# od-liu/CS3602-LLM-Inference-Acceleration

Measured on NVIDIA B200. Metric: kv_compress_step_throughput, higher is better.
Workload: dtype bf16

## Files before the change

### cs3602-llm-inference-acceleration_b200/csrc/kvc_device.cuh

```cuda
#pragma once
#include <cuda_bf16.h>
#include <cuda_fp16.h>
#include <cuda_runtime.h>
#include <stdint.h>

#include <type_traits>

#include "kvc.h"

namespace kvc {

constexpr int kHistBits = 11;
constexpr int kHistBins = 1 << kHistBits;
constexpr int kMiscInts = 128;
constexpr int kMaxPoolHalo = 32;

constexpr int kMiscBin = 0;
constexpr int kMiscBelow = 1;
constexpr int kMiscMaxRaw = 2;
constexpr int kMiscWarpA = 32;
constexpr int kMiscWarpB = 64;
constexpr int kMiscHalo = 96;

struct CarryDev {
    char* acc;
    int64_t asb, ash;
    int32_t group, prev;
};
static_assert(sizeof(CarryDev) == 32, "CarryDev is part of the kernel parameters");

struct LayerDev {
    const char* k_in;
    const char* v_in;
    char* k_out;
    char* v_out;
    int32_t* idx_out;
    const int32_t* idx_in;
    int64_t ksb, ksh, kss;
    int64_t vsb, vsh, vss;
    int32_t S, sink, lo, hi, ksel, tail, score, pool;
    const char* n_in;
    int64_t nsb, nsh;
    CarryDev carry;
};
static_assert(sizeof(LayerDev) == 184, "LayerDev is passed by value in kernel params");

struct BatchDev {
    int32_t B, H;
    int32_t idx_cap;
    int32_t cpr;
    int32_t pad0, pad1;
    int32_t nsw;
    int32_t off_hist, off_idx, off_keys, off_stage;
    int32_t upc;
    char* ws;
    int64_t ws_unit;
    int64_t ws_keys;
    LayerDev layers[KVC_MAX_LAYERS_PER_LAUNCH];
};
static_assert(sizeof(BatchDev) < 32 * 1024, "kernel parameters are limited to 32 KB");

template <int DT>
struct Traits;
template <>
struct Traits<KVC_DTYPE_F32> {
    using Key = uint32_t;
    static constexpr int kElemBytes = 4;
    static constexpr int kKeyBits = 32;
    __device__ static __forceinline__ uint32_t to_raw(float x) { return __float_as_uint(x); }
    __device__ static __forceinline__ float from_raw(uint32_t r) { return __uint_as_float(r); }
    __device__ static __forceinline__ float sumsq(int4 v, float acc) {
        float a = __int_as_float(v.x), b = __int_as_float(v.y), c = __int_as_float(v.z), d = __int_as_float(v.w);
        acc = fmaf(a, a, acc);
        acc = fmaf(b, b, acc);
        acc = fmaf(c, c, acc);
        acc = fmaf(d, d, acc);
        return acc;
    }
};
template <>
struct Traits<KVC_DTYPE_BF16> {
    using Key = uint16_t;
    static constexpr int kElemBytes = 2;
    static constexpr int kKeyBits = 16;
    __device__ static __forceinline__ uint32_t to_raw(float x) {
        return (uint32_t)__bfloat16_as_ushort(__float2bfloat16_rn(x));
    }
    __device__ static __forceinline__ float from_raw(uint32_t r) { return __uint_as_float(r << 16); }
    __device__ static __forceinline__ float sumsq(int4 v, float acc) {
        const uint32_t w[4] = {(uint32_t)v.x, (uint32_t)v.y, (uint32_t)v.z, (uint32_t)v.w};
#pragma unroll
        for (int i = 0; i < 4; ++i) {
            float lo = __uint_as_float(w[i] << 16);
            float hi = __uint_as_float(w[i] & 0xffff0000u);
            acc = fmaf(lo, lo, acc);
            acc = fmaf(hi, hi, acc);
        }
        return acc;
    }
};
template <>
struct Traits<KVC_DTYPE_F16> {
    using Key = uint16_t;
    static constexpr int kElemBytes = 2;
    static constexpr int kKeyBits = 16;
    __device__ static __forceinline__ uint32_t to_raw(float x) {
        return (uint32_t)__half_as_ushort(__float2half_rn(x));
    }
    __device__ static __forceinline__ float from_raw(uint32_t r) {
        return __half2float(__ushort_as_half((unsigned short)r));
    }
    __device__ static __forceinline__ float sumsq(int4 v, float acc) {
        const uint32_t w[4] = {(uint32_t)v.x, (uint32_t)v.y, (uint32_t)v.z, (uint32_t)v.w};
#pragma unroll
        for (int i = 0; i < 4; ++i) {
            float lo = __half2float(__ushort_as_half((unsigned short)(w[i] & 0xffffu)));
            float hi = __half2float(__ushort_as_half((unsigned short)(w[i] >> 16)));
            acc = fmaf(lo, lo, acc);
            acc = fmaf(hi, hi, acc);
        }
        return acc;
    }
};

template <int DT>
__device__ __forceinline__ float round_dt(float x) {
    return Traits<DT>::from_raw(Traits<DT>::to_raw(x));
}

template <typename Key>
__device__ __forceinline__ Key ordered_key(uint32_t raw, bool descending) {
    constexpr int kBits = sizeof(Key) * 8;
    const uint32_t sign = (raw >> (kBits - 1)) & 1u;
    uint32_t k = sign ? ~raw : (raw | (1u << (kBits - 1)));
    if (descending) k = ~k;
    return (Key)k;
}

__device__ __forceinline__ int4 ldg128_stream(const void* p) {
    int4 r;
    asm volatile("ld.global.nc.L1::no_allocate.v4.s32 {%0,%1,%2,%3}, [%4];"
                 : "=r"(r.x), "=r"(r.y), "=r"(r.z), "=r"(r.w)
                 : "l"(p));
    return r;
}
__device__ __forceinline__ void stg128_stream(void* p, int4 v) {
    asm volatile("st.global.L1::no_allocate.v4.s32 [%0], {%1,%2,%3,%4};" ::"l"(p), "r"(v.x), "r"(v.y), "r"(v.z),
                 "r"(v.w)
                 : "memory");
}

__device__ __forceinline__ float group_sum_pow2(float v, int n) {
    for (int o = n >> 1; o > 0; o >>= 1) v += __shfl_xor_sync(0xffffffffu, v, o);
    return v;
}

template <int NT>
__device__ __forceinline__ void find_bin(const uint32_t* hist, int nbins, uint32_t k, int32_t* misc) {
    const int tid = threadIdx.x, lane = tid & 31, warp = tid >> 5;
    const int per = (nbins + NT - 1) / NT;
    const int b0 = tid * per;
    uint32_t loc = 0;
    if ((per & 3) == 0) {
        for (int i = 0; i < per; i += 4) {
            if (b0 + i < nbins) {
                uint4 h = *reinterpret_cast<const uint4*>(hist + b0 + i);
                loc += h.x + h.y + h.z + h.w;
            }
        }
    } else {
        for (int i = 0; i < per; ++i)
            if (b0 + i < nbins) loc += hist[b0 + i];
    }
    uint32_t inc = loc;
#pragma unroll
    for (int o = 1; o < 32; o <<= 1) {
        uint32_t t = __shfl_up_sync(0xffffffffu, inc, o);
        if (lane >= o) inc += t;
    }
    if (lane == 31) misc[kMiscWarpA + warp] = (int32_t)inc;
    __syncthreads();
    uint32_t wbase = 0;
    for (int w = 0; w < warp; ++w) wbase += (uint32_t)misc[kMiscWarpA + w];
    const uint32_t excl = wbase + inc - loc;
    if (excl < k && k <= excl + loc) {
        uint32_t c = excl;
        for (int i = 0; i < per; ++i) {
            const uint32_t h = hist[b0 + i];
            if (c + h >= k) {
                misc[kMiscBin] = b0 + i;
                misc[kMiscBelow] = (int32_t)c;
                break;
            }
            c += h;
        }
    }
    __syncthreads();
}

template <typename Key, int NT>
__device__ __forceinline__ void block_radix_select(const Key* __restrict__ keys, int R, int k, uint32_t* hist,
                                                   int32_t* misc, int32_t* out_idx, int base) {
    constexpr int kBits = sizeof(Key) * 8;
    constexpr int kVec = 16 / sizeof(Key);
// ... 322 lines not shown
```

### cs3602-llm-inference-acceleration_b200/csrc/kvc_fused_tma.cuh

```cuda
#pragma once
#include "kvc_device.cuh"
#include "kvc_tma.cuh"

namespace kvc {

__host__ __device__ constexpr int swz_bits(int cpr) { return (cpr % 8 == 0) ? 3 : (cpr % 4 == 0) ? 2 : (cpr % 2 == 0) ? 1 : 0; }

template <int DT, int CPR>
__device__ __forceinline__ float row_sumsq_smem(uint32_t row_addr, int lane, int cpr) {
    using Tr = Traits<DT>;
    if constexpr (CPR == 0) {
        float tot = 0.f;
        for (int c = 0; c < cpr; ++c) {
            const float a = Tr::sumsq(lds128(row_addr + c * 16), 0.f);
            tot = (c == 0) ? a : tot + a;
        }
        return tot;
    } else {
        constexpr int SB = swz_bits(CPR);
        constexpr int G = 1 << SB;
        const int x = (lane >> (3 - SB)) & (G - 1);
        uint32_t base[G];
#pragma unroll
        for (int m = 0; m < G; ++m) base[m] = row_addr + (uint32_t)(((m ^ x) - m) * 16);
        float acc[CPR];
#pragma unroll
        for (int c = 0; c < CPR; ++c) acc[c] = Tr::sumsq(lds128(base[c & (G - 1)] + c * 16), 0.f);
        float tot = 0.f;
#pragma unroll
        for (int g = 0; g < CPR / G; ++g) {
#pragma unroll
            for (int s = 1; s < G; s <<= 1) {
#pragma unroll
                for (int m = 0; m < G; m += 2 * s) acc[g * G + m] += acc[g * G + m + s];
            }
            tot = (g == 0) ? acc[0] : tot + acc[g * G];
        }
        return tot;
    }
}

__device__ __forceinline__ void warp_load_rows(uint32_t slot, uint32_t bar, const char* src, int rows, bool dense,
                                               int lane, int rb) {
    const bool in = lane < rows;
    const unsigned long long a = (unsigned long long)src;
    const unsigned long long prev = __shfl_up_sync(0xffffffffu, a, 1);
    const bool head = in && (lane == 0 || !dense || a != prev + (unsigned)rb);
    const uint32_t heads = __ballot_sync(0xffffffffu, head);
    if (lane == 0) mbar_arrive_expect_tx(bar, (uint32_t)(rows * rb));
    __syncwarp();
    if (head) {
        const uint32_t later = heads & ~((2u << lane) - 1u);
        const int next = later ? (__ffs(later) - 1) : rows;
        bulk_g2s(slot + (uint32_t)(lane * rb), src, (uint32_t)((next - lane) * rb), bar);
    }
}

struct KeepMap {
    const int32_t* sidx;
    int sink, ksel, tail0;
    __device__ __forceinline__ int operator()(int j) const {
        return j < sink ? j : (j < sink + ksel ? sidx[j - sink] : j + tail0);
    }
};

template <typename Key, int NT>
__device__ __forceinline__ void carry_unit(const CarryDev& c, const KeepMap& src_row, int C, int b, int h) {
    char* base = c.acc + (int64_t)b * c.asb + (int64_t)h * c.group * c.ash;
    const int n = c.group * C;
    for (int e0 = 0; e0 < n; e0 += NT) {
        const int e = e0 + (int)threadIdx.x;
        Key* row = nullptr;
        int i = 0;
        Key val = 0;
        bool write = false;
        if (e < n) {
            const int g = e / C;
            i = e - g * C;
            const int s = src_row(i);
            row = reinterpret_cast<Key*>(base + (int64_t)g * c.ash);
            write = s != i || s >= c.prev;
            if (write && s < c.prev) val = row[s];
        }
        __syncthreads();
        if (write) row[i] = val;
    }
}

__device__ __forceinline__ void gather_unit(const KeepMap& src_row, int C, const char* kbase, const char* vbase,
                                            int64_t kss, int64_t vss, char* ko, char* vo, int rb, uint32_t slot,
                                            uint32_t bar, uint32_t& parity, int stage, int nstage, int lane) {
    const bool kdense = kss == rb, vdense = vss == rb;
    const int nbc = (C + 31) >> 5;
    for (int t = stage; t < 2 * nbc; t += nstage) {
        const bool isv = t >= nbc;
        const int j0 = (isv ? t - nbc : t) << 5;
        const int rows = min(32, C - j0);
        const int row = lane < rows ? src_row(j0 + lane) : 0;
        const char* src = isv ? vbase + (int64_t)row * vss : kbase + (int64_t)row * kss;
        warp_load_rows(slot, bar, src, rows, isv ? vdense : kdense, lane, rb);
        mbar_wait(bar, parity);
        parity ^= 1;
        if (lane == 0) {
            bulk_s2g((isv ? vo : ko) + (int64_t)j0 * rb, slot, (uint32_t)(rows * rb));
            bulk_commit();
            bulk_wait_read<0>();
        }
        __syncwarp();
    }
}

template <int DT, int NT>
__device__ __forceinline__ void keys_from_values(const typename Traits<DT>::Key* src, int R, int score,
                                                 typename Traits<DT>::Key* keys, uint32_t* hist, int32_t* misc) {
    using Tr = Traits<DT>;
    using Key = typename Tr::Key;
    constexpr int kShift0 = Tr::kKeyBits - kHistBits;
    const bool snap = (score == KVC_SCORE_SNAPKV_POOL);
    const bool desc = (score == KVC_SCORE_L2_HIGH);
    uint32_t local_max = 0;
    load_keys_vectorised<DT, NT>(src, R, keys, [&](int i, uint32_t raw) {
        if (snap) {
            keys[i] = (Key)raw;
            local_max = max(local_max, raw);
        } else {
            const Key key = ordered_key<Key>(raw, desc);
            keys[i] = key;
            atomicAdd(&hist[(uint32_t)key >> kShift0], 1u);
        }
    });
    if (snap) {
#pragma unroll
        for (int o = 16; o > 0; o >>= 1) local_max = max(local_max, __shfl_xor_sync(0xffffffffu, local_max, o));
        if ((threadIdx.x & 31) == 0) atomicMax(reinterpret_cast<uint32_t*>(&misc[kMiscMaxRaw]), local_max);
    }
}

template <int DT, int NT, typename Layer>
__device__ __forceinline__ void select_from_memory(const Layer& L, const typename Traits<DT>::Key* norm_row, int b, int bh,
                                                   typename Traits<DT>::Key* keys, uint32_t* hist, int32_t* misc,
                                                   int32_t* sidx) {
    using Key = typename Traits<DT>::Key;
    const int tid = threadIdx.x;
    const int R = L.hi - L.lo;
    if (L.score == KVC_SCORE_GIVEN_INDEX) {
        const int32_t* src = L.idx_in + (int64_t)bh * L.ksel;
        for (int i = tid; i < L.ksel; i += NT) sidx[i] = min(max(src[i], 0), L.S - 1);
        return;
    }
    for (int i = tid; i < kHistBins; i += NT) hist[i] = 0;
    if (tid == 0) misc[kMiscMaxRaw] = 0;
    __syncthreads();
    if (L.score == KVC_SCORE_GIVEN_SCORE || L.score == KVC_SCORE_GIVEN_SCORE_SHARED) {
        const Key* src = reinterpret_cast<const Key*>(L.idx_in) + (int64_t)(L.score == KVC_SCORE_GIVEN_SCORE ? bh : b) * R;
        load_keys_vectorised<DT, NT>(src, R, keys, [&](int i, uint32_t raw) { keys[i] = (Key)raw; });
        __syncthreads();
        snapkv_transform<DT, NT>(keys, R, L.pool, hist, misc, false);
    } else {
        keys_from_values<DT, NT>(norm_row + L.lo, R, L.score, keys, hist, misc);
        __syncthreads();
        if (L.score == KVC_SCORE_SNAPKV_POOL) snapkv_transform<DT, NT>(keys, R, L.pool, hist, misc);
    }
    block_radix_select<Key, NT>(keys, R, L.ksel, hist, misc, sidx, L.lo);
}

template <int DT, int CPR, int NT, int MINB>
__global__ void __launch_bounds__(NT, MINB) kvc_fused_tma_kernel(const __grid_constant__ BatchDev bd) {
    using Tr = Traits<DT>;
    using Key = typename Tr::Key;
    constexpr int kShift0 = Tr::kKeyBits - kHistBits;
    const int cpr = CPR > 0 ? CPR : bd.cpr;
    const int RB = cpr * 16;

    const int bx = blockIdx.x, by = blockIdx.y;
    const LayerDev& L = bd.layers[by];
    const int tid = threadIdx.x, lane = tid & 31, warp = tid >> 5;

    extern __shared__ __align__(128) unsigned char smem[];
    int32_t* misc = reinterpret_cast<int32_t*>(smem);
    uint32_t* hist = reinterpret_cast<uint32_t*>(smem + bd.off_hist);
    int32_t* sidx = reinterpret_cast<int32_t*>(smem + bd.off_idx);
    Key* keys = reinterpret_cast<Key*>(smem + bd.off_keys);
    const int nsw = bd.nsw;
    const bool stager = warp < nsw;
    const uint32_t slot = smem_u32(smem + bd.off_stage) + (uint32_t)(warp * 32 * RB);
    const uint32_t bar = smem_u32(smem + kMiscInts * 4) + (uint32_t)warp * 8;
    uint32_t parity = 0;

    const int R = L.hi - L.lo;
    const int ksel = L.ksel;
    const int score = L.score;
    const bool kdense = L.kss == RB;
    const bool given_score = score == KVC_SCORE_GIVEN_SCORE || score == KVC_SCORE_GIVEN_SCORE_SHARED;
    const bool by_value = given_score || L.n_in != nullptr;
    const bool scan = ksel > 0 && score != KVC_SCORE_GIVEN_INDEX && !by_value;

    if (stager) {
        if (lane == 0) {
            mbar_init(bar, 1);
            mbar_init_fence();
        }
        __syncwarp();
    }
    const int n_units = bd.B * bd.H;
    const int bh_end = min(n_units, (bx + 1) * bd.upc);
    for (int bh = bx * bd.upc; bh < bh_end; ++bh) {
    const int b = bh / bd.H, h = bh - b * bd.H;
    if (bd.ws != nullptr) {
        char* unit = bd.ws + ((int64_t)by * n_units + bh) * bd.ws_unit;
        keys = reinterpret_cast<Key*>(unit);
        sidx = reinterpret_cast<int32_t*>(unit + bd.ws_keys);
    }
    const char* kbase = L.k_in + (int64_t)b * L.ksb + (int64_t)h * L.ksh;
    const char* vbase = L.v_in + (int64_t)b * L.vsb + (int64_t)h * L.vsh;
    const char* kreg = kbase + (int64_t)L.lo * L.kss;
    const int nblk = (R + 31) >> 5;
    if (scan && stager && warp < nblk)
        warp_load_rows(slot, bar, kreg + (int64_t)(warp * 32 + lane) * L.kss, min(32, R - warp * 32), kdense, lane, RB);

    if (ksel > 0 && (score == KVC_SCORE_GIVEN_INDEX || by_value)) {
        const Key* norm_row = L.n_in ? reinterpret_cast<const Key*>(L.n_in + (int64_t)b * L.nsb + (int64_t)h * L.nsh)
                                     : nullptr;
        select_from_memory<DT, NT>(L, norm_row, b, bh, keys, hist, misc, sidx);
    } else if (ksel > 0) {
        for (int i = tid; i < kHistBins; i += NT) hist[i] = 0;
        if (tid == 0) misc[kMiscMaxRaw] = 0;
        __syncthreads();
        const bool snap = (score == KVC_SCORE_SNAPKV_POOL);
        const bool desc = (score == KVC_SCORE_L2_HIGH);
        uint32_t local_max = 0;
        if (stager) {
            for (int blk = warp; blk < nblk; blk += nsw) {
                const int r0 = blk << 5;
                const int rows = min(32, R - r0);
                mbar_wait(bar, parity);
                parity ^= 1;
                float ss = 0.f;
                if (lane < rows) ss = row_sumsq_smem<DT, CPR>(slot + (uint32_t)(lane * RB), lane, cpr);
                __syncwarp();
                const int nb = blk + nsw;
                if (nb < nblk)
                    warp_load_rows(slot, bar, kreg + (int64_t)(nb * 32 + lane) * L.kss, min(32, R - nb * 32), kdense,
                                   lane, RB);
                if (lane < rows) {
                    const uint32_t raw = Tr::to_raw(sqrtf(ss));
                    if (snap) {
                        keys[r0 + lane] = (Key)raw;
                        local_max = max(local_max, raw);
                    } else {
                        const Key key = ordered_key<Key>(raw, desc);
                        keys[r0 + lane] = key;
                        atomicAdd(&hist[(uint32_t)key >> kShift0], 1u);
                    }
                }
            }
        }
        if (snap) {
#pragma unroll
            for (int o = 16; o > 0; o >>= 1) local_max = max(local_max, __shfl_xor_sync(0xffffffffu, local_max, o));
            if (lane == 0) atomicMax(reinterpret_cast<uint32_t*>(&misc[kMiscMaxRaw]), local_max);
        }
        __syncthreads();
        if (snap) snapkv_transform<DT, NT>(keys, R, L.pool, hist, misc);
        block_radix_select<Key, NT>(keys, R, ksel, hist, misc, sidx, L.lo);
    }
    __syncthreads();

    const int C = L.sink + ksel + L.tail;
    const KeepMap src_row{sidx, L.sink, ksel, L.S - L.tail - L.sink - ksel};
    if (L.idx_out != nullptr) {
        int32_t* io = L.idx_out + (int64_t)bh * C;
        for (int j = tid; j < C; j += NT) io[j] = src_row(j);
    }
    if (L.carry.acc != nullptr) carry_unit<Key, NT>(L.carry, src_row, C, b, h);
    if (stager)
        gather_unit(src_row, C, kbase, vbase, L.kss, L.vss, L.k_out + (int64_t)bh * C * RB,
                    L.v_out + (int64_t)bh * C * RB, RB, slot, bar, parity, warp, nsw, lane);
    __syncthreads();
    }
}

}
```

### cs3602-llm-inference-acceleration_b200/csrc/kvc_sm100a.cu

```cuda
#include <algorithm>
#include <atomic>
#include <cstdio>
#include <cmath>
#include <cstdlib>
#include <cstring>
#include <mutex>
#include <type_traits>
#include <utility>
#include <vector>

#include <nvtx3/nvToolsExt.h>

#include "kvc_device.cuh"
#include "kvc_fused_tma.cuh"
#include "kvc_h2o.cuh"
#include "kvc_h2o_tc.cuh"
#include "kvc_slab.cuh"
#include "kvc_vote.cuh"

#ifndef KVC_PART
#define KVC_PART 127
#endif
#define KVC_HAS_CORE (KVC_PART & 1)
#define KVC_HAS_SLAB (KVC_PART & 2)
// ... 474 lines not shown
    bd.idx_cap = s.idx_cap;
    if (lp.ws) {
        bd.ws = (char*)workspace;
        bd.ws_unit = lp.w.unit;
        bd.ws_keys = lp.w.keys;
    }
    bd.nsw = lp.tp.nsw;
    bd.off_hist = lp.tp.off_hist;
    bd.off_idx = lp.tp.off_idx;
    bd.off_keys = lp.tp.off_keys;
    bd.off_stage = lp.tp.off_stage;
    return KVC_OK;
}

template <class Layer>
static void fill_layer_plan(Layer& d, const kvc_layer_plan& p, const kvc_carry_layer* carry, int e) {
    d.S = p.seq_len;
    d.sink = p.sink;
    d.lo = p.sel_lo;
    d.hi = p.sel_hi;
    d.ksel = p.k_sel;
    d.tail = p.tail;
    d.score = p.k_sel > 0 ? p.score : KVC_SCORE_NONE;
    d.pool = p.pool_kernel;
    if (!carry || !carry->acc) return;
    d.carry.acc = (char*)carry->acc;
    d.carry.asb = carry->acc_stride_b * e;
    d.carry.ash = carry->acc_stride_h * e;
    d.carry.group = carry->group;
    d.carry.prev = carry->prev_len < p.seq_len ? carry->prev_len : p.seq_len;
}

}

using namespace kvc;

extern "C" {

#if KVC_HAS_CORE
int kvc_abi_version(void) { return KVC_ABI_VERSION; }

const char* kvc_build_info(void) {
    return "libkvc_sm100a: sm_100a, nvcc " KVC_STR(__CUDACC_VER_MAJOR__) "." KVC_STR(__CUDACC_VER_MINOR__);
}

const char* kvc_status_string(int status) {
    switch (status) {
        case KVC_OK: return "ok";
        case KVC_ERR_INVALID_ARG: return "invalid argument";
        case KVC_ERR_UNSUPPORTED: return "unsupported dtype / head_dim / alignment";
        case KVC_ERR_TOO_LARGE: return "selection region too large for the on-chip score buffer";
        case KVC_ERR_CUDA: return "CUDA error";
        default: return "unknown status";
    }
}

const char* kvc_last_cuda_error(void) { return g_last_error; }

int64_t kvc_launch_count(void) { return g_launches.load(); }

int32_t kvc_max_region_rows(int32_t dtype, int32_t k_sel) {
    if (dtype < 0 || dtype > 2 || k_sel < 0) return 0;
    const int64_t idx = ((int64_t)k_sel + 3) & ~(int64_t)3;
    const int64_t left = (int64_t)kMaxSmemOptin - kSmemFixed - idx * 4;
    if (left <= 0) return 0;
    const int64_t rows = (left & ~(int64_t)15) / key_bytes(dtype);
    return (int32_t)(rows > 0x7fffffff ? 0x7fffffff : rows);
}

int kvc_compress_layers(const kvc_shape* shape, int32_t n_layers, const kvc_layer_plan* plans,
                        const kvc_layer_io* io, void* stream) {
    return kvc_compress_layers_ws(shape, n_layers, plans, io, nullptr, 0, stream);
}

int64_t kvc_workspace_bytes(const kvc_shape* shape, int32_t n_layers, const kvc_layer_plan* plans) {
    int cpr = 0;
    if (check_shape(shape, &cpr) != KVC_OK || n_layers <= 0 || !plans || !row_width_ok(cpr)) return 0;
    const int64_t bh = (int64_t)shape->batch * shape->heads;
    int64_t need = 0;
    for_each_chunk(n_layers, [&](int l0, int nl) -> int {
        const ChunkStats s = chunk_stats(plans + l0, nullptr, nl);
        if (!s.any_select) return KVC_OK;
        const LaunchPlan lp = plan_launch(shape->dtype, cpr, s, false, false, bh * s.n_active,
                                          s.rows_moved / s.n_active * cpr * 16, true);
        if (lp.ws) need = std::max(need, lp.w.unit * bh * s.n_active);
        return KVC_OK;
    });
    return need;
}

int kvc_launch_shape(const kvc_shape* shape, int32_t n_layers, const kvc_layer_plan* plans, int32_t out[4]) {
    int cpr = 0;
    int st = check_shape(shape, &cpr);
    if (st != KVC_OK) return st;
    if (n_layers <= 0 || !plans || !out) return KVC_ERR_INVALID_ARG;
    if (!row_width_ok(cpr)) return KVC_ERR_UNSUPPORTED;
    const ChunkStats s = chunk_stats(plans, nullptr, std::min(n_layers, KVC_MAX_LAYERS_PER_LAUNCH));
    if (s.n_active == 0) return KVC_ERR_INVALID_ARG;
    const int64_t units = (int64_t)shape->batch * shape->heads * s.n_active;
    const LaunchPlan lp = plan_launch(shape->dtype, cpr, s, false, false, units, s.rows_moved / s.n_active * cpr * 16, true);
    if (!lp.tp.ok) return KVC_ERR_TOO_LARGE;
    out[0] = lp.tp.nt;
    out[1] = lp.tp.ctas;
    out[2] = lp.tp.nsw;
    out[3] = lp.ws ? 1 : 0;
    return KVC_OK;
}

int kvc_compress_layers_ws(const kvc_shape* shape, int32_t n_layers, const kvc_layer_plan* plans,
                           const kvc_layer_io* io, void* workspace, int64_t workspace_bytes, void* stream) {
    return kvc_compress_layers_carry(shape, n_layers, plans, io, nullptr, workspace, workspace_bytes, stream);
}

int kvc_compress_layers_carry(const kvc_shape* shape, int32_t n_layers, const kvc_layer_plan* plans,
                              const kvc_layer_io* io, const kvc_carry_layer* carry, void* workspace,
                              int64_t workspace_bytes, void* stream) {
    if (!shape || n_layers < 0 || (n_layers > 0 && (!plans || !io))) return KVC_ERR_INVALID_ARG;
    if (n_layers == 0) return KVC_OK;
    int cpr = 0;
    int st = check_shape(shape, &cpr);
    if (st != KVC_OK) return st;
    if (!row_width_ok(cpr)) return KVC_ERR_UNSUPPORTED;
    const int B = shape->batch, H = shape->heads, dt = shape->dtype;
    const int e = elem_bytes(dt);

    for (int l = 0; l < n_layers; ++l) {
        const kvc_layer_plan& p = plans[l];
        const kvc_layer_io& x = io[l];
        st = check_plan(p, false, x.idx_in != nullptr, x.score_in != nullptr, carry ? carry + l : nullptr, e);
        if (st != KVC_OK) return st;
        const int64_t C = (int64_t)p.sink + p.k_sel + p.tail;
        if (C == 0) continue;
        if (!x.k_in || !x.v_in || !x.k_out || !x.v_out) return KVC_ERR_INVALID_ARG;
        if (C * cpr * 2 > 0x7fffffffLL) return KVC_ERR_TOO_LARGE;
        const uintptr_t a = (uintptr_t)x.k_in | (uintptr_t)x.v_in | (uintptr_t)x.k_out | (uintptr_t)x.v_out;
        if (a & 15) return KVC_ERR_UNSUPPORTED;
        const int64_t s = (x.k_stride_b | x.k_stride_h | x.k_stride_s | x.v_stride_b | x.v_stride_h | x.v_stride_s);
        if ((s * e) & 15) return KVC_ERR_UNSUPPORTED;
    }
    DeviceGuard guard(shape->device);
    NvtxRange nvtx_range("kvc_compress_layers_ws");
    if (guard.status != KVC_OK) return guard.status;

    return for_each_chunk(n_layers, [&](int l0, int nl) -> int {
        const ChunkStats s = chunk_stats(plans + l0, io + l0, nl);
        if (s.n_active == 0) return KVC_OK;
        const bool light = s.any_select && !s.any_scan;
        const LaunchPlan lp = plan_launch(dt, cpr, s, light, false, (int64_t)B * H * s.n_active,
                                          s.rows_moved / s.n_active * cpr * 16, workspace != nullptr);
        BatchDev bd;
        int st = fill_batch(bd, shape, cpr, s, lp, workspace, workspace_bytes);
        if (st != KVC_OK) return st;
        bd.upc = lp.tp.upc;
        int m = 0;
        for (int l = l0; l < l0 + nl; ++l) {
            const kvc_layer_plan& p = plans[l];
            const kvc_layer_io& x = io[l];
            if (p.sink + p.k_sel + p.tail == 0) continue;
            LayerDev& d = bd.layers[m++];
            d.k_in = (const char*)x.k_in;
            d.v_in = (const char*)x.v_in;
            d.k_out = (char*)x.k_out;
            d.v_out = (char*)x.v_out;
            d.idx_out = x.idx_out;
            d.idx_in = (p.score == KVC_SCORE_GIVEN_SCORE || p.score == KVC_SCORE_GIVEN_SCORE_SHARED) ? (const int32_t*)x.score_in
                                                                                              : x.idx_in;
            d.ksb = x.k_stride_b * e;
            d.ksh = x.k_stride_h * e;
            d.kss = x.k_stride_s * e;
            d.vsb = x.v_stride_b * e;
            d.vsh = x.v_stride_h * e;
            d.vss = x.v_stride_s * e;
            if (ranked(p) && x.norms_in) {
                d.n_in = (const char*)x.norms_in;
                d.nsb = x.n_stride_b * key_bytes(dt);
                d.nsh = x.n_stride_h * key_bytes(dt);
            }
            fill_layer_plan(d, p, carry ? carry + l : nullptr, e);
        }
        FusedFn fn = pick_tma(dt, cpr, lp.tp.nt);
        dim3 grid((unsigned)(((int64_t)B * H + lp.tp.upc - 1) / lp.tp.upc), (unsigned)s.n_active, 1);
        st = ensure_tma_attrs((const void*)fn, shape->device);
        if (st != KVC_OK) return st;
        fn<<<grid, lp.tp.nt, lp.tp.smem, (cudaStream_t)stream>>>(bd);
        return launched("kvc_fused_tma_kernel launch");
    });
}

int kvc_key_norms(const kvc_shape* shape, const void* k_in, int64_t stride_b, int64_t stride_h, int64_t stride_s,
                  int32_t row_lo, int32_t row_hi, void* norms_out, void* stream) {
    if (!shape || !k_in || !norms_out || row_lo < 0 || row_hi < row_lo) return KVC_ERR_INVALID_ARG;
    const int B = shape->batch, H = shape->heads, D = shape->head_dim, dt = shape->dtype;
    if (B <= 0 || H <= 0 || D <= 0) return KVC_ERR_INVALID_ARG;
    if (dt != KVC_DTYPE_F32 && dt != KVC_DTYPE_F16 && dt != KVC_DTYPE_BF16) return KVC_ERR_UNSUPPORTED;
    const int e = elem_bytes(dt);
    if (((int64_t)D * e) % 16 != 0 || ((uintptr_t)k_in & 15)) return KVC_ERR_UNSUPPORTED;
    if (((stride_b | stride_h | stride_s) * e) & 15) return KVC_ERR_UNSUPPORTED;
    const int R = row_hi - row_lo;
    const int64_t total = (int64_t)B * H * R;
    if (total == 0) return KVC_OK;
    DeviceGuard guard(shape->device);
    NvtxRange nvtx_range("kvc_key_norms");
    if (guard.status != KVC_OK) return guard.status;
    const int cpr = D * e / 16;
    const int lpr = pow2_lanes(cpr), cpl = cpr / lpr;
    const int rpw = 32 / lpr;
    const int64_t warps_needed = (total + rpw - 1) / rpw;
    int64_t blocks = (warps_needed + 7) / 8;
    const int64_t cap = 148LL * 8 * 4;
    if (blocks > cap) blocks = cap;
    cudaStream_t s = (cudaStream_t)stream;
    const int64_t sb = stride_b * e, sh = stride_h * e, ss = stride_s * e;
    by_dtype(dt, [&](auto d) {
        kvc_norm_kernel<d><<<(unsigned)blocks, 256, 0, s>>>((const char*)k_in, sb, sh, ss, H, row_lo, R, total, lpr, cpl,
                                                            (typename Traits<d>::Key*)norms_out);
    });
    return launched("kvc_norm_kernel launch");
}

int kvc_select(int32_t dtype, int32_t device, const void* scores, int64_t n_rows, int32_t n, int32_t k,
               int32_t largest, int32_t* idx_out, void* stream) {
    if (!scores || !idx_out || n_rows < 0 || n < 0 || k < 0 || k > n) return KVC_ERR_INVALID_ARG;
    if (dtype != KVC_DTYPE_F32 && dtype != KVC_DTYPE_F16 && dtype != KVC_DTYPE_BF16) return KVC_ERR_UNSUPPORTED;
    if (n_rows == 0 || k == 0) return KVC_OK;
    if (n_rows > 0x7fffffffLL) return KVC_ERR_INVALID_ARG;
    const size_t smem = fused_smem_bytes(dtype, n, (k + 3) & ~3);
    if (smem > (size_t)kMaxSmemOptin) return KVC_ERR_TOO_LARGE;
    DeviceGuard guard(device);
    NvtxRange nvtx_range("kvc_select");
    if (guard.status != KVC_OK) return guard.status;
    return by_dtype(dtype, [&](auto d) -> int {
        const int st = ensure_smem((const void*)kvc_select_kernel<d, kNT>, smem);
        if (st != KVC_OK) return st;
        kvc_select_kernel<d, kNT><<<(unsigned)n_rows, kNT, smem, (cudaStream_t)stream>>>(
            (const typename Traits<d>::Key*)scores, n, k, largest, idx_out);
        return launched("kvc_select_kernel launch");
    });
}

#endif

#if KVC_HAS_SLAB
int kvc_slab_append(const kvc_shape* shape, int32_t n_layers, const kvc_slab_layer* slabs,
                    const kvc_slab_new_rows* rows, void* stream) {
    int cpr = 0;
    int st = check_shape(shape, &cpr);
    if (st != KVC_OK) return st;
    if (n_layers < 0 || (n_layers > 0 && (!slabs || !rows))) return KVC_ERR_INVALID_ARG;
    if (n_layers == 0) return KVC_OK;
    if (!row_width_ok(cpr)) return KVC_ERR_UNSUPPORTED;
    const int B = shape->batch, H = shape->heads, dt = shape->dtype;
    const int e = elem_bytes(dt);
    for (int l = 0; l < n_layers; ++l) {
        const kvc_slab_layer& sl = slabs[l];
        const kvc_slab_new_rows& r = rows[l];
        if (r.n_new < 0 || r.cur_len < 0) return KVC_ERR_INVALID_ARG;
        if (r.n_new == 0) continue;
        if (!sl.k || !sl.v || !sl.norms || !r.k_new || !r.v_new) return KVC_ERR_INVALID_ARG;
        const uintptr_t a = (uintptr_t)sl.k | (uintptr_t)sl.v | (uintptr_t)r.k_new | (uintptr_t)r.v_new;
        if (a & 15) return KVC_ERR_UNSUPPORTED;
        const int64_t sb = sl.k_stride_b | sl.k_stride_h | sl.v_stride_b | sl.v_stride_h | r.k_stride_b | r.k_stride_h |
                           r.k_stride_s | r.v_stride_b | r.v_stride_h | r.v_stride_s;
        if ((sb * e) & 15) return KVC_ERR_UNSUPPORTED;
        if ((int64_t)B * H * r.n_new > 0x7fffffffLL) return KVC_ERR_TOO_LARGE;
    }
    DeviceGuard guard(shape->device);
    NvtxRange nvtx_range("kvc_slab_append");
    if (guard.status != KVC_OK) return guard.status;
    auto fill = [&](AppendLayerDev& d, const kvc_slab_layer& sl, const kvc_slab_new_rows& r) {
        d.k_new = (const char*)r.k_new;
        d.v_new = (const char*)r.v_new;
        d.k = (char*)sl.k;
        d.v = (char*)sl.v;
        d.n = (char*)sl.norms;
        d.nksb = r.k_stride_b * e;
        d.nksh = r.k_stride_h * e;
        d.nkss = r.k_stride_s * e;
        d.nvsb = r.v_stride_b * e;
        d.nvsh = r.v_stride_h * e;
        d.nvss = r.v_stride_s * e;
        d.ksb = sl.k_stride_b * e;
        d.ksh = sl.k_stride_h * e;
        d.vsb = sl.v_stride_b * e;
        d.vsh = sl.v_stride_h * e;
        d.nsb = sl.n_stride_b * key_bytes(dt);
        d.nsh = sl.n_stride_h * key_bytes(dt);
        d.cur_len = r.cur_len;
        d.n_new = r.n_new;
    };
    if (n_layers == 1 && rows[0].n_new > 0 && rows[0].n_new < 32) {
        AppendOneDev one;
        one.B = B;
        one.H = H;
        one.max_new = rows[0].n_new;
        one.cpr = cpr;
        fill(one.layers[0], slabs[0], rows[0]);
        const int64_t threads = (int64_t)B * H * rows[0].n_new;
        pick_append_one(dt, cpr)<<<(unsigned)((threads + 127) / 128), 128, 0, (cudaStream_t)stream>>>(one);
        return launched("kvc_slab_append_kernel launch");
    }
    AppendFn fn = pick_append(dt, cpr);
    return for_each_chunk(n_layers, [&](int l0, int nl) -> int {
        AppendBatchDev bd;
        memset(&bd, 0, sizeof(bd));
        bd.B = B;
        bd.H = H;
        int n_active = 0, max_new = 0;
        for (int l = 0; l < nl; ++l) {
            const kvc_slab_layer& sl = slabs[l0 + l];
            const kvc_slab_new_rows& r = rows[l0 + l];
            if (r.n_new == 0) continue;
            fill(bd.layers[n_active++], sl, r);
            if (r.n_new > max_new) max_new = r.n_new;
        }
        if (n_active == 0) return KVC_OK;
        bd.max_new = max_new;
        bd.cpr = cpr;
        if (max_new >= 32) {
            AppendFn tfn = pick_append_tma(dt, cpr);
            const int st = ensure_tma_attrs((const void*)tfn, shape->device);
            if (st != KVC_OK) return st;
            const size_t smem = 128 + (size_t)8 * 32 * cpr * 16;
            const int64_t items = (int64_t)B * H * ((max_new + 31) / 32);
            int64_t blocks = (items + 7) / 8;
            const int64_t cap = 148LL * 3 * 8;
            if (blocks > cap) blocks = cap;
            dim3 grid((unsigned)blocks, (unsigned)n_active, 1);
            tfn<<<grid, 256, smem, (cudaStream_t)stream>>>(bd);
        } else {
            const int64_t threads = (int64_t)B * H * max_new;
            dim3 grid((unsigned)((threads + 127) / 128), (unsigned)n_active, 1);
            fn<<<grid, 128, 0, (cudaStream_t)stream>>>(bd);
        }
        return launched("kvc_slab_append_kernel launch");
    });
}

// ... 555 lines not shown
```

### cs3602-llm-inference-acceleration_b200/csrc/kvc_tma.cuh

```cuda
#pragma once
#include <cuda_runtime.h>
#include <stdint.h>

namespace kvc {

__device__ __forceinline__ uint32_t smem_u32(const void* p) { return (uint32_t)__cvta_generic_to_shared(p); }

__device__ __forceinline__ void mbar_init(uint32_t bar, uint32_t count) {
    asm volatile("mbarrier.init.shared::cta.b64 [%0], %1;" ::"r"(bar), "r"(count) : "memory");
}
__device__ __forceinline__ void mbar_init_fence() { asm volatile("fence.mbarrier_init.release.cluster;" ::: "memory"); }

__device__ __forceinline__ void mbar_arrive_expect_tx(uint32_t bar, uint32_t bytes) {
    asm volatile("mbarrier.arrive.expect_tx.shared::cta.b64 _, [%0], %1;" ::"r"(bar), "r"(bytes) : "memory");
}

__device__ __forceinline__ bool mbar_try_wait(uint32_t bar, uint32_t parity) {
    uint32_t ok;
    asm volatile(
        "{\n\t.reg .pred p;\n\t"
        "mbarrier.try_wait.parity.shared::cta.b64 p, [%1], %2;\n\t"
        "selp.u32 %0, 1, 0, p;\n\t}"
        : "=r"(ok)
        : "r"(bar), "r"(parity)
        : "memory");
    return ok != 0;
}
__device__ __forceinline__ void mbar_wait(uint32_t bar, uint32_t parity) {
    while (!mbar_try_wait(bar, parity)) {
    }
}

__device__ __forceinline__ void bulk_g2s(uint32_t dst_smem, const void* src_gmem, uint32_t bytes, uint32_t bar) {
    asm volatile("cp.async.bulk.shared::cluster.global.mbarrier::complete_tx::bytes [%0], [%1], %2, [%3];" ::"r"(dst_smem),
                 "l"(src_gmem), "r"(bytes), "r"(bar)
                 : "memory");
}
__device__ __forceinline__ void bulk_s2g(void* dst_gmem, uint32_t src_smem, uint32_t bytes) {
    asm volatile("cp.async.bulk.global.shared::cta.bulk_group [%0], [%1], %2;" ::"l"(dst_gmem), "r"(src_smem), "r"(bytes)
                 : "memory");
}
__device__ __forceinline__ void bulk_commit() { asm volatile("cp.async.bulk.commit_group;" ::: "memory"); }
template <int N>
__device__ __forceinline__ void bulk_wait_read() {
    asm volatile("cp.async.bulk.wait_group.read %0;" ::"n"(N) : "memory");
}
__device__ __forceinline__ void fence_proxy_async_smem() { asm volatile("fence.proxy.async.shared::cta;" ::: "memory"); }

__device__ __forceinline__ int4 lds128(uint32_t addr) {
    int4 r;
    asm volatile("ld.shared.v4.s32 {%0,%1,%2,%3}, [%4];" : "=r"(r.x), "=r"(r.y), "=r"(r.z), "=r"(r.w) : "r"(addr));
    return r;
}

}
```

Measured before the change: 6446.

## Hold best-scored key rows in spare shared memory to skip re-reading them in gather

During the L2-norm scan, each stager warp keeps the top-scoring K rows (up to a hold count sized from spare shared memory) in a per-warp shared store. After selection, the kept indices are mapped to the held rows by binary search, and the gather stage copies those rows from shared memory instead of issuing bulk global loads. It only applies when CPR equals 10 with no workspace. The cost is extra shared memory, which can reduce occupancy, plus warp-serial replacement loops during the scan.

```diff
diff --git a/cs3602-llm-inference-acceleration_b200/csrc/kvc_device.cuh b/cs3602-llm-inference-acceleration_b200/csrc/kvc_device.cuh
--- a/cs3602-llm-inference-acceleration_b200/csrc/kvc_device.cuh
+++ b/cs3602-llm-inference-acceleration_b200/csrc/kvc_device.cuh
@@ -49,7 +49,8 @@
     int32_t B, H;
     int32_t idx_cap;
     int32_t cpr;
-    int32_t pad0, pad1;
+    int32_t lab_flags;
+    int32_t hold;
     int32_t nsw;
     int32_t off_hist, off_idx, off_keys, off_stage;
     int32_t upc;
diff --git a/cs3602-llm-inference-acceleration_b200/csrc/kvc_fused_tma.cuh b/cs3602-llm-inference-acceleration_b200/csrc/kvc_fused_tma.cuh
--- a/cs3602-llm-inference-acceleration_b200/csrc/kvc_fused_tma.cuh
+++ b/cs3602-llm-inference-acceleration_b200/csrc/kvc_fused_tma.cuh
@@ -87,9 +87,65 @@
     }
 }
 
+#ifdef KVC_LAB
+constexpr int kLabSkipKeptK = 1;
+#endif
+
+__device__ __forceinline__ void warp_load_some_rows(uint32_t slot, uint32_t bar, const char* src, bool want, bool dense,
+                                                    int lane, int rb) {
+    const unsigned long long a = (unsigned long long)src;
+    const unsigned long long prev = __shfl_up_sync(0xffffffffu, a, 1);
+    const uint32_t wants = __ballot_sync(0xffffffffu, want);
+    const bool prev_want = lane > 0 && ((wants >> (lane - 1)) & 1u);
+    const bool head = want && (!prev_want || !dense || a != prev + (unsigned)rb);
+    const uint32_t cont = __ballot_sync(0xffffffffu, want && !head);
+    if (lane == 0) mbar_arrive_expect_tx(bar, (uint32_t)(__popc(wants) * rb));
+    __syncwarp();
+    if (head) {
+        const uint32_t brk = ~cont & ~((2u << lane) - 1u);
+        const int next = brk ? (__ffs(brk) - 1) : 32;
+        bulk_g2s(slot + (uint32_t)(lane * rb), src, (uint32_t)((next - lane) * rb), bar);
+    }
+}
+
+__device__ __forceinline__ uint32_t warp_max_u32(uint32_t v) {
+#pragma unroll
+    for (int o = 16; o > 0; o >>= 1) v = max(v, __shfl_xor_sync(0xffffffffu, v, o));
+    return v;
+}
+
+constexpr int kHoldCpr = 10;
+
+__device__ __forceinline__ void hold_rows(uint32_t key, bool in, int row, uint32_t slot, uint32_t store, int hold,
+                                          int cpr, int rb, int lane, uint32_t& skey, int& srow) {
+    uint32_t thr = warp_max_u32(lane < hold ? skey : 0u);
+    uint32_t cand = __ballot_sync(0xffffffffu, in && key < thr);
+    while (cand) {
+        const int c = __ffs(cand) - 1;
+        cand &= cand - 1;
+        const uint32_t ck = __shfl_sync(0xffffffffu, key, c);
+        const int cr = __shfl_sync(0xffffffffu, row, c);
+        if (ck >= thr) continue;
+        const int s = __ffs(__ballot_sync(0xffffffffu, lane < hold && skey == thr)) - 1;
+        if (lane < cpr) sts128(store + (uint32_t)(s * rb + lane * 16), lds128(slot + (uint32_t)(c * rb + lane * 16)));
+        if (lane == s) {
+            skey = ck;
+            srow = cr;
+        }
+        thr = warp_max_u32(lane < hold ? skey : 0u);
+    }
+}
+
+struct HeldRows {
+    const int16_t* map = nullptr;
+    uint32_t store = 0;
+    int sel0 = 0, nsel = 0;
+};
+
 __device__ __forceinline__ void gather_unit(const KeepMap& src_row, int C, const char* kbase, const char* vbase,
                                             int64_t kss, int64_t vss, char* ko, char* vo, int rb, uint32_t slot,
-                                            uint32_t bar, uint32_t& parity, int stage, int nstage, int lane) {
+                                            uint32_t bar, uint32_t& parity, int stage, int nstage, int lane,
+                                            const HeldRows& held = HeldRows{}) {
     const bool kdense = kss == rb, vdense = vss == rb;
     const int nbc = (C + 31) >> 5;
     for (int t = stage; t < 2 * nbc; t += nstage) {
@@ -98,7 +154,20 @@
         const int rows = min(32, C - j0);
         const int row = lane < rows ? src_row(j0 + lane) : 0;
         const char* src = isv ? vbase + (int64_t)row * vss : kbase + (int64_t)row * kss;
-        warp_load_rows(slot, bar, src, rows, isv ? vdense : kdense, lane, rb);
+        const bool from_store = !isv && held.nsel > 0 && j0 < held.sel0 + held.nsel && j0 + 32 > held.sel0;
+        if (from_store) {
+            const int i = j0 + lane - held.sel0;
+            const int hs = (lane < rows && i >= 0 && i < held.nsel) ? (held.map ? held.map[i] : 0) : -1;
+            warp_load_some_rows(slot, bar, src, lane < rows && hs < 0, kdense, lane, rb);
+            if (held.map && hs >= 0) {
+                for (int c = 0; c < rb; c += 16)
+                    sts128(slot + (uint32_t)(lane * rb + c), lds128(held.store + (uint32_t)(hs * rb + c)));
+                fence_proxy_async_smem();
+            }
+            __syncwarp();
+        } else {
+            warp_load_rows(slot, bar, src, rows, isv ? vdense : kdense, lane, rb);
+        }
         mbar_wait(bar, parity);
         parity ^= 1;
         if (lane == 0) {
@@ -194,6 +263,10 @@
     const bool given_score = score == KVC_SCORE_GIVEN_SCORE || score == KVC_SCORE_GIVEN_SCORE_SHARED;
     const bool by_value = given_score || L.n_in != nullptr;
     const bool scan = ksel > 0 && score != KVC_SCORE_GIVEN_INDEX && !by_value;
+    const bool hold = CPR == kHoldCpr && bd.hold > 0 && bd.ws == nullptr && scan &&
+                      (score == KVC_SCORE_L2_LOW || score == KVC_SCORE_L2_HIGH);
+    const uint32_t hstore = smem_u32(smem + bd.off_stage) + (uint32_t)(nsw * 32 * RB);
+    int32_t* hrow = reinterpret_cast<int32_t*>(smem + bd.off_stage + nsw * 32 * RB + nsw * bd.hold * RB);
 
     if (stager) {
         if (lane == 0) {
@@ -230,6 +303,8 @@
         const bool desc = (score == KVC_SCORE_L2_HIGH);
         uint32_t local_max = 0;
         if (stager) {
+            uint32_t skey = 0xffffffffu;
+            int srow = -1;
             for (int blk = warp; blk < nblk; blk += nsw) {
                 const int r0 = blk << 5;
                 const int rows = min(32, R - r0);
@@ -237,6 +312,13 @@
                 parity ^= 1;
                 float ss = 0.f;
                 if (lane < rows) ss = row_sumsq_smem<DT, CPR>(slot + (uint32_t)(lane * RB), lane, cpr);
+                if constexpr (CPR == kHoldCpr) {
+                    if (hold) {
+                        const uint32_t key = lane < rows ? (uint32_t)ordered_key<Key>(Tr::to_raw(sqrtf(ss)), desc) : 0u;
+                        hold_rows(key, lane < rows, L.lo + r0 + lane, slot, hstore + (uint32_t)(warp * bd.hold * RB),
+                                  bd.hold, cpr, RB, lane, skey, srow);
+                    }
+                }
                 __syncwarp();
                 const int nb = blk + nsw;
                 if (nb < nblk)
@@ -254,6 +336,7 @@
                     }
                 }
             }
+            if (hold && lane < bd.hold) hrow[warp * bd.hold + lane] = srow;
         }
         if (snap) {
 #pragma unroll
@@ -273,9 +356,31 @@
         for (int j = tid; j < C; j += NT) io[j] = src_row(j);
     }
     if (L.carry.acc != nullptr) carry_unit<Key, NT>(L.carry, src_row, C, b, h);
+    HeldRows held;
+    if (hold) {
+        int16_t* map = reinterpret_cast<int16_t*>(keys);
+        for (int i = tid; i < ksel; i += NT) map[i] = -1;
+        __syncthreads();
+        for (int e = tid; e < nsw * bd.hold; e += NT) {
+            const int r = hrow[e];
+            if (r < 0) continue;
+            int lo = 0, hi = ksel;
+            while (lo < hi) {
+                const int mid = (lo + hi) >> 1;
+                if (sidx[mid] < r) lo = mid + 1;
+                else hi = mid;
+            }
+            if (lo < ksel && sidx[lo] == r) map[lo] = (int16_t)e;
+        }
+        __syncthreads();
+        held = HeldRows{map, hstore, L.sink, ksel};
+    }
+#ifdef KVC_LAB
+    if (scan && (bd.lab_flags & kLabSkipKeptK)) held = HeldRows{nullptr, 0, L.sink, ksel};
+#endif
     if (stager)
         gather_unit(src_row, C, kbase, vbase, L.kss, L.vss, L.k_out + (int64_t)bh * C * RB,
-                    L.v_out + (int64_t)bh * C * RB, RB, slot, bar, parity, warp, nsw, lane);
+                    L.v_out + (int64_t)bh * C * RB, RB, slot, bar, parity, warp, nsw, lane, held);
     __syncthreads();
     }
 }
diff --git a/cs3602-llm-inference-acceleration_b200/csrc/kvc_sm100a.cu b/cs3602-llm-inference-acceleration_b200/csrc/kvc_sm100a.cu
--- a/cs3602-llm-inference-acceleration_b200/csrc/kvc_sm100a.cu
+++ b/cs3602-llm-inference-acceleration_b200/csrc/kvc_sm100a.cu
@@ -650,6 +650,17 @@
         int st = fill_batch(bd, shape, cpr, s, lp, workspace, workspace_bytes);
         if (st != KVC_OK) return st;
         bd.upc = lp.tp.upc;
+        size_t smem = lp.tp.smem;
+        if (cpr == kHoldCpr && s.any_scan && !lp.ws) {
+            const int limit = std::min(kSmemPerSM / lp.tp.ctas - 1024, kMaxSmemOptin);
+            const int per_row = lp.tp.nsw * (cpr * 16 + 4);
+            const int spare = limit - (int)lp.tp.smem;
+            bd.hold = std::min(32, spare > 0 ? spare / per_row : 0);
+            smem += (size_t)bd.hold * per_row;
+        }
+#ifdef KVC_LAB
+        bd.lab_flags = env_int("KVC_LAB_SKIP_KEPT_K", 0) ? kLabSkipKeptK : 0;
+#endif
         int m = 0;
         for (int l = l0; l < l0 + nl; ++l) {
             const kvc_layer_plan& p = plans[l];
@@ -680,7 +691,7 @@
         dim3 grid((unsigned)(((int64_t)B * H + lp.tp.upc - 1) / lp.tp.upc), (unsigned)s.n_active, 1);
         st = ensure_tma_attrs((const void*)fn, shape->device);
         if (st != KVC_OK) return st;
-        fn<<<grid, lp.tp.nt, lp.tp.smem, (cudaStream_t)stream>>>(bd);
+        fn<<<grid, lp.tp.nt, smem, (cudaStream_t)stream>>>(bd);
         return launched("kvc_fused_tma_kernel launch");
     });
 }
diff --git a/cs3602-llm-inference-acceleration_b200/csrc/kvc_tma.cuh b/cs3602-llm-inference-acceleration_b200/csrc/kvc_tma.cuh
--- a/cs3602-llm-inference-acceleration_b200/csrc/kvc_tma.cuh
+++ b/cs3602-llm-inference-acceleration_b200/csrc/kvc_tma.cuh
@@ -52,5 +52,8 @@
     asm volatile("ld.shared.v4.s32 {%0,%1,%2,%3}, [%4];" : "=r"(r.x), "=r"(r.y), "=r"(r.z), "=r"(r.w) : "r"(addr));
     return r;
 }
+__device__ __forceinline__ void sts128(uint32_t addr, int4 v) {
+    asm volatile("st.shared.v4.s32 [%0], {%1,%2,%3,%4};" ::"r"(addr), "r"(v.x), "r"(v.y), "r"(v.z), "r"(v.w) : "memory");
+}
 
 }
```

Result: slower. 6104 (median of 6 runs) (-5.3%).
